# facebookresearch/vsc2022

Hardware: AMD Instinct MI355X
Metric: query-videos localized/sec @ 512-d SSCD (higher is better)
Workload: dtype fp32 results; int8 / fp16 MFMA pre-filters; 1 GPU; BASELINE configs[3]: full pipeline incl. score normalisation + TN localisation, 40000 query videos split over 1 GPU(s), 2000000 reference + 2000000 noise frames; query_videos_per_gpu=40000, query_frames_per_gpu=1000000, ref_frames=2000000, dim=512, global_k=48000000, candidates=1000000, pairs_localized=200000, matches=446939, hits=48000000, score_normalisation_in_step=True, parallelism=single GPU

## Files before the change

vsc2022_amd/csrc/radix.h:

```cpp
#pragma once
#include "vscmi_common.h"

namespace vscmi {

constexpr int RADIX_ITEMS = 16;
constexpr int RADIX_TILE = 256 * RADIX_ITEMS;

template <class K>
__device__ __forceinline__ unsigned radix_digit(K key, int shift, bool desc) {
    if (desc) key = ~key;
    return (unsigned)(key >> shift) & 255u;
}

template <class K>
__global__ __launch_bounds__(256) void radix_hist_kernel(const K* __restrict__ keys, int64_t n, int shift, bool desc,
                                                         unsigned* __restrict__ hist, int ntiles) {
    __shared__ unsigned h[256];
    h[threadIdx.x] = 0;
    __syncthreads();
    const int64_t base = (int64_t)blockIdx.x * RADIX_TILE;
#pragma unroll 4
    for (int k = 0; k < RADIX_ITEMS; ++k) {
        const int64_t e = base + k * 256 + threadIdx.x;
        if (e < n) atomicAdd(&h[radix_digit(keys[e], shift, desc)], 1u);
    }
    __syncthreads();
    hist[(int64_t)threadIdx.x * ntiles + blockIdx.x] = h[threadIdx.x];
}

__global__ __launch_bounds__(256) void radix_scan_rows_kernel(unsigned* __restrict__ hist, int ntiles,
                                                              unsigned* __restrict__ totals) {
    __shared__ unsigned part[256];
    unsigned* row = hist + (int64_t)blockIdx.x * ntiles;
    const int per = (ntiles + 255) / 256;
    const int t0 = threadIdx.x * per;
    unsigned s = 0;
    for (int t = t0; t < min(ntiles, t0 + per); ++t) s += row[t];
    part[threadIdx.x] = s;
    __syncthreads();
    for (int off = 1; off < 256; off <<= 1) {
        const unsigned v = threadIdx.x >= off ? part[threadIdx.x - off] : 0u;
        __syncthreads();
        part[threadIdx.x] += v;
        __syncthreads();
    }
    unsigned run = threadIdx.x ? part[threadIdx.x - 1] : 0u;
    for (int t = t0; t < min(ntiles, t0 + per); ++t) {
        const unsigned c = row[t];
        row[t] = run;
        run += c;
    }
    if (threadIdx.x == 255) totals[blockIdx.x] = part[255];
}

__global__ __launch_bounds__(256) void radix_scan_totals_kernel(unsigned* __restrict__ totals) {
    __shared__ unsigned part[256];
    part[threadIdx.x] = totals[threadIdx.x];
    __syncthreads();
    for (int off = 1; off < 256; off <<= 1) {
        const unsigned v = threadIdx.x >= off ? part[threadIdx.x - off] : 0u;
        __syncthreads();
        part[threadIdx.x] += v;
        __syncthreads();
    }
    totals[threadIdx.x] = threadIdx.x ? part[threadIdx.x - 1] : 0u;
}

template <class K, class V>
__global__ __launch_bounds__(256) void radix_scatter_kernel(const K* __restrict__ keys_in, const V* __restrict__ vals_in,
                                                            K* __restrict__ keys_out, V* __restrict__ vals_out, int64_t n,
                                                            int shift, bool desc, const unsigned* __restrict__ hist,
                                                            const unsigned* __restrict__ totals, int ntiles) {
    __shared__ unsigned wcount[4][256];
    __shared__ unsigned dstart[256];
    __shared__ unsigned gbase[256];
    __shared__ K skey[RADIX_TILE];
    __shared__ V sval[RADIX_TILE];
    const int lane = threadIdx.x & 63, wave = threadIdx.x >> 6;
    for (int x = threadIdx.x; x < 4 * 256; x += 256) (&wcount[0][0])[x] = 0;
    gbase[threadIdx.x] = totals[threadIdx.x] + hist[(int64_t)threadIdx.x * ntiles + blockIdx.x];
    __syncthreads();
    const int64_t tile0 = (int64_t)blockIdx.x * RADIX_TILE;
    const int64_t base = tile0 + (int64_t)wave * (RADIX_ITEMS * 64);
    K key[RADIX_ITEMS];
    unsigned rank[RADIX_ITEMS];
#pragma unroll
    for (int k = 0; k < RADIX_ITEMS; ++k) {
        const int64_t e = base + k * 64 + lane;
        const bool valid = e < n;
        key[k] = valid ? keys_in[e] : (K)0;
        const unsigned d = radix_digit(key[k], shift, desc);
        unsigned long long peers = __ballot(valid);
#pragma unroll
        for (int b = 0; b < 8; ++b) {
            const unsigned long long m = __ballot((d >> b) & 1u);
            peers &= ((d >> b) & 1u) ? m : ~m;
        }
        const unsigned before = (unsigned)__popcll(peers & ((1ull << lane) - 1));
        unsigned c = 0;
        if (valid) c = wcount[wave][d];
        __builtin_amdgcn_wave_barrier();
        if (valid && before == 0) wcount[wave][d] = c + (unsigned)__popcll(peers);
        __builtin_amdgcn_wave_barrier();
        rank[k] = c + before;
    }
    __syncthreads();
    {
        const int d = threadIdx.x;
        unsigned run = 0;
#pragma unroll
        for (int w = 0; w < 4; ++w) {
            const unsigned c = wcount[w][d];
            wcount[w][d] = run;
            run += c;
        }
        dstart[d] = run;
    }
    __syncthreads();
    for (int off = 1; off < 256; off <<= 1) {
        const unsigned v = threadIdx.x >= off ? dstart[threadIdx.x - off] : 0u;
        __syncthreads();
        dstart[threadIdx.x] += v;
        __syncthreads();
    }
    const unsigned mine_incl = dstart[threadIdx.x];
    const unsigned prev_incl = threadIdx.x ? dstart[threadIdx.x - 1] : 0u;
    __syncthreads();
    dstart[threadIdx.x] = prev_incl;
    (void)mine_incl;
    __syncthreads();
#pragma unroll
    for (int k = 0; k < RADIX_ITEMS; ++k) {
        const int64_t e = base + k * 64 + lane;
        if (e < n) {
            const unsigned d = radix_digit(key[k], shift, desc);
            const unsigned slot = dstart[d] + wcount[wave][d] + rank[k];
            skey[slot] = key[k];
            sval[slot] = vals_in[e];
        }
    }
    __syncthreads();
    const int cnt = (int)min((int64_t)RADIX_TILE, n - tile0);
#pragma unroll 4
    for (int k = 0; k < RADIX_ITEMS; ++k) {
        const int slot = k * 256 + threadIdx.x;
        if (slot < cnt) {
            const K kk = skey[slot];
            const unsigned d = radix_digit(kk, shift, desc);
            const int64_t pos = (int64_t)gbase[d] + (slot - dstart[d]);
            keys_out[pos] = kk;
            vals_out[pos] = sval[slot];
        }
    }
}

inline size_t radix_tmp_bytes(int64_t n) {
    const int64_t ntiles = (n + RADIX_TILE - 1) / RADIX_TILE;
    return (size_t)(256 * ntiles + 256) * sizeof(unsigned);
}

template <class K, class V>
int radix_sort_pairs(K* keys_a, K* keys_b, V* vals_a, V* vals_b, int64_t n, int begin_bit, int end_bit, bool desc,
                     void* tmp, hipStream_t stream, int begin2 = 0, int end2 = 0) {
    if (n <= 0) return 0;
    if (n > 0xffffffffLL) {
        set_error("radix_sort_pairs: %lld entries exceed the 2^32 limit of the sort", (long long)n);
        return -1;
    }
    const int ntiles = (int)((n + RADIX_TILE - 1) / RADIX_TILE);
    unsigned* hist = reinterpret_cast<unsigned*>(tmp);
    unsigned* totals = hist + (size_t)256 * ntiles;
    int where = 0;
    for (int pass = 0;; ++pass) {
        const int n1 = (end_bit - begin_bit + 7) / 8;
        const int shift = pass < n1 ? begin_bit + 8 * pass : begin2 + 8 * (pass - n1);
        if (pass >= n1 && shift >= end2) break;
        const K* ki = where ? keys_b : keys_a;
        const V* vi = where ? vals_b : vals_a;
        K* ko = where ? keys_a : keys_b;
        V* vo = where ? vals_a : vals_b;
        hipLaunchKernelGGL((radix_hist_kernel<K>), dim3((unsigned)ntiles), dim3(256), 0, stream, ki, n, shift, desc, hist, ntiles);
        hipLaunchKernelGGL(radix_scan_rows_kernel, dim3(256), dim3(256), 0, stream, hist, ntiles, totals);
        hipLaunchKernelGGL(radix_scan_totals_kernel, dim3(1), dim3(256), 0, stream, totals);
        hipLaunchKernelGGL((radix_scatter_kernel<K, V>), dim3((unsigned)ntiles), dim3(256), 0, stream, ki, vi, ko, vo, n, shift,
                           desc, hist, totals, ntiles);
        if (hipGetLastError() != hipSuccess) return -1;
        where ^= 1;
    }
    return where;
}

}
```

Before: 19880 query-videos/s.

## Rework radix sort: XCD tile mapping, fused scan, atomic ranking, small-n path

Rewrites the radix sort kernels. Tiles are mapped to blocks so that each XCD gets a contiguous range. The histogram kernel uses vectorized key loads. The two scan kernels are merged into one, with a last-block ticket finishing the totals scan. The scatter kernel uses 8 waves and ranks keys with LDS atomic peer masks instead of 8 ballots per key, and it stages keys and values through a single shared buffer. A new single-block kernel sorts inputs of up to 12288 entries in one launch covering all passes. This aims to cut launch count, LDS footprint and ranking cost, at the price of more complex synchronization and a risk of correctness problems in the atomic ranking.

Result: faster. 20170 query-videos/s (median of 6 runs) (+1.4%).

```diff
diff --git a/vsc2022_amd/csrc/radix.h b/vsc2022_amd/csrc/radix.h
--- a/vsc2022_amd/csrc/radix.h
+++ b/vsc2022_amd/csrc/radix.h
@@ -3,8 +3,18 @@
 
 namespace vscmi {
 
-constexpr int RADIX_ITEMS = 16;
-constexpr int RADIX_TILE = 256 * RADIX_ITEMS;
+constexpr int RADIX_TILE = 4096;
+constexpr int RADIX_XCDS = 8;
+constexpr int RADIX_HIST_THREADS = 256;
+constexpr int RADIX_SCAN_THREADS = 1024;
+constexpr int RADIX_SCAN_SHORT_ROW = 1024;
+constexpr int RADIX_WAVES = 8;
+constexpr int RADIX_THREADS = 64 * RADIX_WAVES;
+constexpr int RADIX_ITEMS = RADIX_TILE / RADIX_THREADS;
+constexpr int RADIX_SMALL_WAVES = 16;
+constexpr int RADIX_SMALL_THREADS = 64 * RADIX_SMALL_WAVES;
+constexpr int RADIX_SMALL_BATCH = 4;
+constexpr int64_t RADIX_SMALL_N = 12288;
 
 template <class K>
 __device__ __forceinline__ unsigned radix_digit(K key, int shift, bool desc) {
@@ -12,151 +22,393 @@
     return (unsigned)(key >> shift) & 255u;
 }
 
+__host__ __device__ __forceinline__ int radix_pass_shift(int pass, int begin_bit, int end_bit, int begin2, int end2) {
+    const int n1 = (end_bit - begin_bit + 7) / 8;
+    if (pass < n1) return begin_bit + 8 * pass;
+    const int shift = begin2 + 8 * (pass - n1);
+    return shift < end2 ? shift : -1;
+}
+
+__host__ __device__ __forceinline__ int radix_small_segment(int n) {
+    return (n + RADIX_SMALL_THREADS - 1) / RADIX_SMALL_THREADS * 64;
+}
+
+__device__ __forceinline__ void radix_wave_order() {
+    __builtin_amdgcn_fence(__ATOMIC_ACQ_REL, "wavefront");
+    __builtin_amdgcn_wave_barrier();
+}
+
+__device__ __forceinline__ unsigned long long radix_peers(unsigned long long* mask, unsigned d, bool valid, int lane) {
+    const unsigned long long me = 1ull << lane;
+    if (valid) atomicOr(&mask[d], me);
+    radix_wave_order();
+    unsigned long long peers = 0;
+    if (valid) peers = __hip_atomic_load(&mask[d], __ATOMIC_RELAXED, __HIP_MEMORY_SCOPE_WORKGROUP);
+    radix_wave_order();
+    if (valid) atomicAnd(&mask[d], ~me);
+    radix_wave_order();
+    return peers;
+}
+
+__device__ __forceinline__ unsigned radix_lanes_below(unsigned long long m) {
+    return __builtin_amdgcn_mbcnt_hi((unsigned)(m >> 32), __builtin_amdgcn_mbcnt_lo((unsigned)m, 0u));
+}
+
+__device__ __forceinline__ unsigned radix_rank_issue(unsigned* counter, unsigned long long peers, unsigned d, bool valid, unsigned* who) {
+    const unsigned before = radix_lanes_below(peers);
+    *who = ((unsigned)(__ffsll((long long)peers) - 1) & 63u) << 8 | before;
+    unsigned c = 0;
+    if (valid && before == 0) c = atomicAdd(&counter[d], (unsigned)__popcll(peers));
+    radix_wave_order();
+    return c;
+}
+
+__device__ __forceinline__ unsigned radix_rank_finish(unsigned c, unsigned who) {
+    return (unsigned)__shfl((int)c, (int)(who >> 8)) + (who & 255u);
+}
+
+__device__ __forceinline__ int radix_tile_of_block(int block, int ntiles) {
+    const int per = ntiles / RADIX_XCDS, rem = ntiles % RADIX_XCDS;
+    const int x = block % RADIX_XCDS, y = block / RADIX_XCDS;
+    return x * per + min(x, rem) + y;
+}
+
+__device__ __forceinline__ unsigned radix_wave_incl_scan(unsigned v, int lane) {
+#pragma unroll
+    for (int off = 1; off < 64; off <<= 1) {
+        const unsigned u = (unsigned)__shfl_up((int)v, off);
+        if (lane >= off) v += u;
+    }
+    return v;
+}
+
 template <class K>
-__global__ __launch_bounds__(256) void radix_hist_kernel(const K* __restrict__ keys, int64_t n, int shift, bool desc,
-                                                         unsigned* __restrict__ hist, int ntiles) {
+__global__ __launch_bounds__(RADIX_HIST_THREADS) void radix_hist_kernel(const K* __restrict__ keys, int64_t n, int shift, bool desc,
+                                                                        unsigned* __restrict__ hist, int ntiles,
+                                                                        unsigned* __restrict__ ticket) {
+    constexpr int VEC = 16 / (int)sizeof(K);
+    struct alignas(16) KeyVec { K k[VEC]; };
     __shared__ unsigned h[256];
     h[threadIdx.x] = 0;
-    __syncthreads();
-    const int64_t base = (int64_t)blockIdx.x * RADIX_TILE;
+    if (blockIdx.x == 0 && threadIdx.x == 0) *ticket = 0;
+    __syncthreads();
+    const int tile = radix_tile_of_block((int)blockIdx.x, ntiles);
+    const int64_t base = (int64_t)tile * RADIX_TILE;
+    if (base + RADIX_TILE <= n && (reinterpret_cast<uintptr_t>(keys) & 15u) == 0) {
+        const KeyVec* kv = reinterpret_cast<const KeyVec*>(keys + base);
+#pragma unroll
+        for (int k = 0; k < RADIX_TILE / VEC / RADIX_HIST_THREADS; ++k) {
+            const KeyVec v = kv[k * RADIX_HIST_THREADS + threadIdx.x];
+#pragma unroll
+            for (int u = 0; u < VEC; ++u) atomicAdd(&h[radix_digit(v.k[u], shift, desc)], 1u);
+        }
+    } else {
 #pragma unroll 4
-    for (int k = 0; k < RADIX_ITEMS; ++k) {
-        const int64_t e = base + k * 256 + threadIdx.x;
-        if (e < n) atomicAdd(&h[radix_digit(keys[e], shift, desc)], 1u);
-    }
-    __syncthreads();
-    hist[(int64_t)threadIdx.x * ntiles + blockIdx.x] = h[threadIdx.x];
-}
-
-__global__ __launch_bounds__(256) void radix_scan_rows_kernel(unsigned* __restrict__ hist, int ntiles,
-                                                              unsigned* __restrict__ totals) {
-    __shared__ unsigned part[256];
+        for (int k = 0; k < RADIX_TILE / RADIX_HIST_THREADS; ++k) {
+            const int64_t e = base + k * RADIX_HIST_THREADS + threadIdx.x;
+            if (e < n) atomicAdd(&h[radix_digit(keys[e], shift, desc)], 1u);
+        }
+    }
+    __syncthreads();
+    hist[(int64_t)threadIdx.x * ntiles + tile] = h[threadIdx.x];
+}
+
+template <int THREADS>
+__global__ __launch_bounds__(THREADS) void radix_scan_kernel(unsigned* __restrict__ hist, int ntiles, unsigned* totals,
+                                                             unsigned* ticket) {
+    constexpr int WAVES = THREADS / 64;
+    constexpr int GROUP = 4;
+    __shared__ unsigned wsum[WAVES < 4 ? 4 : WAVES];
+    __shared__ unsigned last;
+    const int lane = threadIdx.x & 63;
+    const int wave = __builtin_amdgcn_readfirstlane((int)(threadIdx.x >> 6));
     unsigned* row = hist + (int64_t)blockIdx.x * ntiles;
-    const int per = (ntiles + 255) / 256;
-    const int t0 = threadIdx.x * per;
+    const int seg = (ntiles + 64 * WAVES - 1) / (64 * WAVES) * 64;
+    const int lo = min(ntiles, wave * seg), hi = min(ntiles, lo + seg);
     unsigned s = 0;
-    for (int t = t0; t < min(ntiles, t0 + per); ++t) s += row[t];
-    part[threadIdx.x] = s;
-    __syncthreads();
-    for (int off = 1; off < 256; off <<= 1) {
-        const unsigned v = threadIdx.x >= off ? part[threadIdx.x - off] : 0u;
-        __syncthreads();
-        part[threadIdx.x] += v;
-        __syncthreads();
-    }
-    unsigned run = threadIdx.x ? part[threadIdx.x - 1] : 0u;
-    for (int t = t0; t < min(ntiles, t0 + per); ++t) {
-        const unsigned c = row[t];
-        row[t] = run;
-        run += c;
-    }
-    if (threadIdx.x == 255) totals[blockIdx.x] = part[255];
-}
-
-__global__ __launch_bounds__(256) void radix_scan_totals_kernel(unsigned* __restrict__ totals) {
-    __shared__ unsigned part[256];
-    part[threadIdx.x] = totals[threadIdx.x];
-    __syncthreads();
-    for (int off = 1; off < 256; off <<= 1) {
-        const unsigned v = threadIdx.x >= off ? part[threadIdx.x - off] : 0u;
-        __syncthreads();
-        part[threadIdx.x] += v;
-        __syncthreads();
-    }
-    totals[threadIdx.x] = threadIdx.x ? part[threadIdx.x - 1] : 0u;
+#pragma unroll 4
+    for (int t = lo + lane; t < hi; t += 64) s += row[t];
+#pragma unroll
+    for (int off = 32; off >= 1; off >>= 1) s += (unsigned)__shfl_xor((int)s, off);
+    if (lane == 0) wsum[wave] = s;
+    __syncthreads();
+    unsigned carry = 0, total = 0;
+#pragma unroll
+    for (int w = 0; w < WAVES; ++w) {
+        const unsigned c = wsum[w];
+        if (w < wave) carry += c;
+        total += c;
+    }
+    for (int t0 = lo; t0 < hi; t0 += 64 * GROUP) {
+        unsigned c[GROUP];
+#pragma unroll
+        for (int g = 0; g < GROUP; ++g) {
+            const int t = t0 + g * 64 + lane;
+            c[g] = t < hi ? row[t] : 0u;
+        }
+#pragma unroll
+        for (int g = 0; g < GROUP; ++g) {
+            const int t = t0 + g * 64 + lane;
+            const unsigned incl = radix_wave_incl_scan(c[g], lane);
+            if (t < hi) row[t] = carry + incl - c[g];
+            carry += (unsigned)__shfl((int)incl, 63);
+        }
+    }
+    if (threadIdx.x == 0) {
+        __hip_atomic_store(&totals[blockIdx.x], total, __ATOMIC_RELAXED, __HIP_MEMORY_SCOPE_AGENT);
+        __threadfence();
+        last = atomicAdd(ticket, 1u) == gridDim.x - 1 ? 1u : 0u;
+    }
+    __syncthreads();
+    if (!last) return;
+    __threadfence();
+    unsigned v = 0;
+    if (threadIdx.x < 256) v = __hip_atomic_load(&totals[threadIdx.x], __ATOMIC_RELAXED, __HIP_MEMORY_SCOPE_AGENT);
+    const unsigned incl = radix_wave_incl_scan(v, lane);
+    if (lane == 63) wsum[wave] = incl;
+    __syncthreads();
+    if (threadIdx.x < 256) {
+        unsigned excl = incl - v;
+        for (int w = 0; w < wave; ++w) excl += wsum[w];
+        totals[threadIdx.x] = excl;
+    }
 }
 
 template <class K, class V>
-__global__ __launch_bounds__(256) void radix_scatter_kernel(const K* __restrict__ keys_in, const V* __restrict__ vals_in,
-                                                            K* __restrict__ keys_out, V* __restrict__ vals_out, int64_t n,
-                                                            int shift, bool desc, const unsigned* __restrict__ hist,
-                                                            const unsigned* __restrict__ totals, int ntiles) {
-    __shared__ unsigned wcount[4][256];
-    __shared__ unsigned dstart[256];
-    __shared__ unsigned gbase[256];
-    __shared__ K skey[RADIX_TILE];
-    __shared__ V sval[RADIX_TILE];
+__global__ __launch_bounds__(RADIX_THREADS) void radix_scatter_kernel(const K* __restrict__ keys_in, const V* __restrict__ vals_in,
+                                                                      K* __restrict__ keys_out, V* __restrict__ vals_out, int64_t n,
+                                                                      int shift, bool desc, const unsigned* __restrict__ hist,
+                                                                      const unsigned* __restrict__ totals, int ntiles) {
+    constexpr int ESZ = sizeof(K) > sizeof(V) ? (int)sizeof(K) : (int)sizeof(V);
+    __shared__ unsigned wcount[RADIX_WAVES][256];
+    __shared__ unsigned gdelta[256];
+    __shared__ unsigned wsum[4];
+    __shared__ __attribute__((aligned(16))) unsigned char stage[RADIX_TILE * ESZ];
+    K* skey = reinterpret_cast<K*>(stage);
+    V* sval = reinterpret_cast<V*>(stage);
     const int lane = threadIdx.x & 63, wave = threadIdx.x >> 6;
-    for (int x = threadIdx.x; x < 4 * 256; x += 256) (&wcount[0][0])[x] = 0;
-    gbase[threadIdx.x] = totals[threadIdx.x] + hist[(int64_t)threadIdx.x * ntiles + blockIdx.x];
-    __syncthreads();
-    const int64_t tile0 = (int64_t)blockIdx.x * RADIX_TILE;
+    for (int x = threadIdx.x; x < RADIX_WAVES * 256; x += RADIX_THREADS) (&wcount[0][0])[x] = 0;
+    static_assert(RADIX_TILE * ESZ >= RADIX_WAVES * 256 * 8, "the waves' lane masks live in the staging buffer");
+    for (int x = threadIdx.x; x < RADIX_WAVES * 256; x += RADIX_THREADS) reinterpret_cast<unsigned long long*>(stage)[x] = 0ull;
+    const int tile = radix_tile_of_block((int)blockIdx.x, ntiles);
+    unsigned gbase = 0;
+    if (threadIdx.x < 256) gbase = totals[threadIdx.x] + hist[(int64_t)threadIdx.x * ntiles + tile];
+    const int64_t tile0 = (int64_t)tile * RADIX_TILE;
     const int64_t base = tile0 + (int64_t)wave * (RADIX_ITEMS * 64);
     K key[RADIX_ITEMS];
-    unsigned rank[RADIX_ITEMS];
+    V val[RADIX_ITEMS];
+    unsigned slot[RADIX_ITEMS];
 #pragma unroll
     for (int k = 0; k < RADIX_ITEMS; ++k) {
         const int64_t e = base + k * 64 + lane;
-        const bool valid = e < n;
-        key[k] = valid ? keys_in[e] : (K)0;
-        const unsigned d = radix_digit(key[k], shift, desc);
-        unsigned long long peers = __ballot(valid);
-#pragma unroll
-        for (int b = 0; b < 8; ++b) {
-            const unsigned long long m = __ballot((d >> b) & 1u);
-            peers &= ((d >> b) & 1u) ? m : ~m;
-        }
-        const unsigned before = (unsigned)__popcll(peers & ((1ull << lane) - 1));
-        unsigned c = 0;
-        if (valid) c = wcount[wave][d];
-        __builtin_amdgcn_wave_barrier();
-        if (valid && before == 0) wcount[wave][d] = c + (unsigned)__popcll(peers);
-        __builtin_amdgcn_wave_barrier();
-        rank[k] = c + before;
-    }
-    __syncthreads();
-    {
-        const int d = threadIdx.x;
-        unsigned run = 0;
-#pragma unroll
-        for (int w = 0; w < 4; ++w) {
-            const unsigned c = wcount[w][d];
-            wcount[w][d] = run;
-            run += c;
-        }
-        dstart[d] = run;
-    }
-    __syncthreads();
-    for (int off = 1; off < 256; off <<= 1) {
-        const unsigned v = threadIdx.x >= off ? dstart[threadIdx.x - off] : 0u;
-        __syncthreads();
-        dstart[threadIdx.x] += v;
-        __syncthreads();
-    }
-    const unsigned mine_incl = dstart[threadIdx.x];
-    const unsigned prev_incl = threadIdx.x ? dstart[threadIdx.x - 1] : 0u;
-    __syncthreads();
-    dstart[threadIdx.x] = prev_incl;
-    (void)mine_incl;
-    __syncthreads();
+        key[k] = e < n ? keys_in[e] : (K)0;
+    }
 #pragma unroll
     for (int k = 0; k < RADIX_ITEMS; ++k) {
         const int64_t e = base + k * 64 + lane;
-        if (e < n) {
-            const unsigned d = radix_digit(key[k], shift, desc);
-            const unsigned slot = dstart[d] + wcount[wave][d] + rank[k];
-            skey[slot] = key[k];
-            sval[slot] = vals_in[e];
+        val[k] = e < n ? vals_in[e] : (V)0;
+    }
+    __syncthreads();
+    {
+        unsigned long long* mask = reinterpret_cast<unsigned long long*>(stage) + wave * 256;
+        unsigned long long peers[RADIX_ITEMS];
+        unsigned who[RADIX_ITEMS];
+#pragma unroll
+        for (int k = 0; k < RADIX_ITEMS; ++k)
+            peers[k] = radix_peers(mask, radix_digit(key[k], shift, desc), base + k * 64 + lane < n, lane);
+#pragma unroll
+        for (int k = 0; k < RADIX_ITEMS; ++k)
+            slot[k] = radix_rank_issue(wcount[wave], peers[k], radix_digit(key[k], shift, desc), base + k * 64 + lane < n, &who[k]);
+#pragma unroll
+        for (int k = 0; k < RADIX_ITEMS; ++k) slot[k] = radix_rank_finish(slot[k], who[k]);
+    }
+    __syncthreads();
+    unsigned tot = 0;
+    if (threadIdx.x < 256) {
+#pragma unroll
+        for (int w = 0; w < RADIX_WAVES; ++w) {
+            const unsigned c = wcount[w][threadIdx.x];
+            wcount[w][threadIdx.x] = tot;
+            tot += c;
+        }
+    }
+    const unsigned incl = radix_wave_incl_scan(tot, lane);
+    if (lane == 63 && wave < 4) wsum[wave] = incl;
+    __syncthreads();
+    if (threadIdx.x < 256) {
+        unsigned start = incl - tot;
+        for (int w = 0; w < wave; ++w) start += wsum[w];
+#pragma unroll
+        for (int w = 0; w < RADIX_WAVES; ++w) wcount[w][threadIdx.x] += start;
+        gdelta[threadIdx.x] = gbase - start;
+    }
+    __syncthreads();
+#pragma unroll
+    for (int k = 0; k < RADIX_ITEMS; ++k) {
+        if (base + k * 64 + lane < n) {
+            slot[k] += wcount[wave][radix_digit(key[k], shift, desc)];
+            skey[slot[k]] = key[k];
         }
     }
     __syncthreads();
     const int cnt = (int)min((int64_t)RADIX_TILE, n - tile0);
+    unsigned pos[RADIX_ITEMS];
+#pragma unroll
+    for (int k = 0; k < RADIX_ITEMS; ++k) {
+        const int s = k * RADIX_THREADS + threadIdx.x;
+        pos[k] = 0;
+        if (s < cnt) {
+            const K kk = skey[s];
+            pos[k] = gdelta[radix_digit(kk, shift, desc)] + (unsigned)s;
+            keys_out[pos[k]] = kk;
+        }
+    }
+    __syncthreads();
+#pragma unroll
+    for (int k = 0; k < RADIX_ITEMS; ++k)
+        if (base + k * 64 + lane < n) sval[slot[k]] = val[k];
+    __syncthreads();
+#pragma unroll
+    for (int k = 0; k < RADIX_ITEMS; ++k) {
+        const int s = k * RADIX_THREADS + threadIdx.x;
+        if (s < cnt) vals_out[pos[k]] = sval[s];
+    }
+}
+
+template <class K, class V>
+__global__ __launch_bounds__(RADIX_SMALL_THREADS) void radix_small_kernel(K* keys_a, K* keys_b, V* vals_a, V* vals_b, int n, int begin_bit,
+                                                                          int end_bit, int begin2, int end2, bool desc) {
+    __shared__ unsigned wcount[RADIX_SMALL_WAVES][256];
+    __shared__ unsigned long long wmask[RADIX_SMALL_WAVES][256];
+    __shared__ unsigned wsum[4];
+    const int lane = threadIdx.x & 63;
+    const int wave = __builtin_amdgcn_readfirstlane((int)(threadIdx.x >> 6));
+    for (int x = threadIdx.x; x < RADIX_SMALL_WAVES * 256; x += RADIX_SMALL_THREADS) (&wmask[0][0])[x] = 0ull;
+    const int seg = radix_small_segment(n);
+    const int lo = min(n, wave * seg), hi = min(n, lo + seg);
+    unsigned* counter = wcount[wave];
+    for (int pass = 0;; ++pass) {
+        const int shift = radix_pass_shift(pass, begin_bit, end_bit, begin2, end2);
+        if (shift < 0) break;
+        const K* ki = (pass & 1) ? keys_b : keys_a;
+        const V* vi = (pass & 1) ? vals_b : vals_a;
+        K* ko = (pass & 1) ? keys_a : keys_b;
+        V* vo = (pass & 1) ? vals_a : vals_b;
+        for (int x = threadIdx.x; x < RADIX_SMALL_WAVES * 256; x += RADIX_SMALL_THREADS) (&wcount[0][0])[x] = 0;
+        __syncthreads();
 #pragma unroll 4
-    for (int k = 0; k < RADIX_ITEMS; ++k) {
-        const int slot = k * 256 + threadIdx.x;
-        if (slot < cnt) {
-            const K kk = skey[slot];
-            const unsigned d = radix_digit(kk, shift, desc);
-            const int64_t pos = (int64_t)gbase[d] + (slot - dstart[d]);
-            keys_out[pos] = kk;
-            vals_out[pos] = sval[slot];
-        }
-    }
-}
-
-inline size_t radix_tmp_bytes(int64_t n) {
-    const int64_t ntiles = (n + RADIX_TILE - 1) / RADIX_TILE;
-    return (size_t)(256 * ntiles + 256) * sizeof(unsigned);
+        for (int e = lo + lane; e < hi; e += 64) atomicAdd(&counter[radix_digit(ki[e], shift, desc)], 1u);
+        __syncthreads();
+        unsigned tot = 0;
+        if (threadIdx.x < 256) {
+#pragma unroll
+            for (int w = 0; w < RADIX_SMALL_WAVES; ++w) {
+                const unsigned c = wcount[w][threadIdx.x];
+                wcount[w][threadIdx.x] = tot;
+                tot += c;
+            }
+        }
+        const unsigned incl = radix_wave_incl_scan(tot, lane);
+        if (lane == 63 && wave < 4) wsum[wave] = incl;
+        __syncthreads();
+        if (threadIdx.x < 256) {
+            unsigned start = incl - tot;
+            for (int w = 0; w < wave; ++w) start += wsum[w];
+#pragma unroll
+            for (int w = 0; w < RADIX_SMALL_WAVES; ++w) wcount[w][threadIdx.x] += start;
+        }
+        __syncthreads();
+        for (int e0 = lo; e0 < hi; e0 += 64 * RADIX_SMALL_BATCH) {
+            K key[RADIX_SMALL_BATCH];
+            V val[RADIX_SMALL_BATCH];
+#pragma unroll
+            for (int b = 0; b < RADIX_SMALL_BATCH; ++b) {
+                const int e = e0 + b * 64 + lane;
+                key[b] = e < hi ? ki[e] : (K)0;
+                val[b] = e < hi ? vi[e] : (V)0;
+            }
+            unsigned long long peers[RADIX_SMALL_BATCH];
+            unsigned c[RADIX_SMALL_BATCH], who[RADIX_SMALL_BATCH];
+#pragma unroll
+            for (int b = 0; b < RADIX_SMALL_BATCH; ++b)
+                peers[b] = radix_peers(wmask[wave], radix_digit(key[b], shift, desc), e0 + b * 64 + lane < hi, lane);
+#pragma unroll
+            for (int b = 0; b < RADIX_SMALL_BATCH; ++b)
+                c[b] = radix_rank_issue(counter, peers[b], radix_digit(key[b], shift, desc), e0 + b * 64 + lane < hi, &who[b]);
+#pragma unroll
+            for (int b = 0; b < RADIX_SMALL_BATCH; ++b) {
+                const bool valid = e0 + b * 64 + lane < hi;
+                const unsigned pos = radix_rank_finish(c[b], who[b]);
+                if (valid) {
+                    ko[pos] = key[b];
+                    vo[pos] = val[b];
+                }
+            }
+        }
+        __threadfence_block();
+        __syncthreads();
+    }
+}
+
+struct RadixTmpLayout {
+    int64_t ntiles, hist, totals, ticket, words;
+};
+
+inline RadixTmpLayout radix_tmp_layout(int64_t n) {
+    RadixTmpLayout t;
+    t.ntiles = (n + RADIX_TILE - 1) / RADIX_TILE;
+    t.hist = 0;
+    t.totals = t.hist + 256 * t.ntiles;
+    t.ticket = t.totals + 256;
+    t.words = t.ticket + 1;
+    return t;
+}
+
+inline size_t radix_tmp_bytes(int64_t n) { return (size_t)radix_tmp_layout(n).words * sizeof(unsigned); }
+
+inline bool radix_use_small(int64_t n) { return n <= RADIX_SMALL_N; }
+
+template <class K, class V>
+int radix_sort_pairs_tiled(K* keys_a, K* keys_b, V* vals_a, V* vals_b, int64_t n, int begin_bit, int end_bit, bool desc,
+                           void* tmp, hipStream_t stream, int begin2 = 0, int end2 = 0) {
+    const RadixTmpLayout lay = radix_tmp_layout(n);
+    const int ntiles = (int)lay.ntiles;
+    unsigned* hist = reinterpret_cast<unsigned*>(tmp) + lay.hist;
+    unsigned* totals = reinterpret_cast<unsigned*>(tmp) + lay.totals;
+    unsigned* ticket = reinterpret_cast<unsigned*>(tmp) + lay.ticket;
+    int where = 0;
+    for (int pass = 0;; ++pass) {
+        const int shift = radix_pass_shift(pass, begin_bit, end_bit, begin2, end2);
+        if (shift < 0) break;
+        const K* ki = where ? keys_b : keys_a;
+        const V* vi = where ? vals_b : vals_a;
+        K* ko = where ? keys_a : keys_b;
+        V* vo = where ? vals_a : vals_b;
+        hipLaunchKernelGGL((radix_hist_kernel<K>), dim3((unsigned)ntiles), dim3(RADIX_HIST_THREADS), 0, stream, ki, n, shift, desc,
+                           hist, ntiles, ticket);
+        if (ntiles <= RADIX_SCAN_SHORT_ROW)
+            hipLaunchKernelGGL((radix_scan_kernel<256>), dim3(256), dim3(256), 0, stream, hist, ntiles, totals, ticket);
+        else
+            hipLaunchKernelGGL((radix_scan_kernel<RADIX_SCAN_THREADS>), dim3(256), dim3(RADIX_SCAN_THREADS), 0, stream, hist, ntiles,
+                               totals, ticket);
+        hipLaunchKernelGGL((radix_scatter_kernel<K, V>), dim3((unsigned)ntiles), dim3(RADIX_THREADS), 0, stream, ki, vi, ko, vo, n,
+                           shift, desc, hist, totals, ntiles);
+        if (hipGetLastError() != hipSuccess) return -1;
+        where ^= 1;
+    }
+    return where;
+}
+
+template <class K, class V>
+int radix_sort_pairs_small(K* keys_a, K* keys_b, V* vals_a, V* vals_b, int64_t n, int begin_bit, int end_bit, bool desc,
+                           hipStream_t stream, int begin2 = 0, int end2 = 0) {
+    int passes = 0;
+    while (radix_pass_shift(passes, begin_bit, end_bit, begin2, end2) >= 0) ++passes;
+    if (passes == 0) return 0;
+    hipLaunchKernelGGL((radix_small_kernel<K, V>), dim3(1), dim3(RADIX_SMALL_THREADS), 0, stream, keys_a, keys_b, vals_a, vals_b,
+                       (int)n, begin_bit, end_bit, begin2, end2, desc);
+    if (hipGetLastError() != hipSuccess) return -1;
+    return passes & 1;
 }
 
 template <class K, class V>
@@ -167,27 +419,8 @@
         set_error("radix_sort_pairs: %lld entries exceed the 2^32 limit of the sort", (long long)n);
         return -1;
     }
-    const int ntiles = (int)((n + RADIX_TILE - 1) / RADIX_TILE);
-    unsigned* hist = reinterpret_cast<unsigned*>(tmp);
-    unsigned* totals = hist + (size_t)256 * ntiles;
-    int where = 0;
-    for (int pass = 0;; ++pass) {
-        const int n1 = (end_bit - begin_bit + 7) / 8;
-        const int shift = pass < n1 ? begin_bit + 8 * pass : begin2 + 8 * (pass - n1);
-        if (pass >= n1 && shift >= end2) break;
-        const K* ki = where ? keys_b : keys_a;
-        const V* vi = where ? vals_b : vals_a;
-        K* ko = where ? keys_a : keys_b;
-        V* vo = where ? vals_a : vals_b;
-        hipLaunchKernelGGL((radix_hist_kernel<K>), dim3((unsigned)ntiles), dim3(256), 0, stream, ki, n, shift, desc, hist, ntiles);
-        hipLaunchKernelGGL(radix_scan_rows_kernel, dim3(256), dim3(256), 0, stream, hist, ntiles, totals);
-        hipLaunchKernelGGL(radix_scan_totals_kernel, dim3(1), dim3(256), 0, stream, totals);
-        hipLaunchKernelGGL((radix_scatter_kernel<K, V>), dim3((unsigned)ntiles), dim3(256), 0, stream, ki, vi, ko, vo, n, shift,
-                           desc, hist, totals, ntiles);
-        if (hipGetLastError() != hipSuccess) return -1;
-        where ^= 1;
-    }
-    return where;
-}
-
-}
+    if (radix_use_small(n)) return radix_sort_pairs_small<K, V>(keys_a, keys_b, vals_a, vals_b, n, begin_bit, end_bit, desc, stream, begin2, end2);
+    return radix_sort_pairs_tiled<K, V>(keys_a, keys_b, vals_a, vals_b, n, begin_bit, end_bit, desc, tmp, stream, begin2, end2);
+}
+
+}
```
